# NeuroDiffGym/neurodiffeq

Measured on NVIDIA H100. Metric: collocation-points/sec (residual+grad), higher is better.
Workload: dtype f32

## Files before the change

### neurodiffeq_b200/csrc/pinnjet_common.cuh

```cuda
#pragma once
#include <cuda_runtime.h>
#include <stdint.h>
#include <stdlib.h>
#include "pinnjet_plan.h"

namespace pj {

inline bool pdl_enabled() {
    static const int on = [] {
        const char* e = getenv("PINNJET_PDL");
        return (e && e[0] == '1') ? 1 : 0;
    }();
    return on != 0;
}

template <typename... KArgs, typename... Args>
inline cudaError_t launch_kernel(void (*kern)(KArgs...), dim3 grid, dim3 block, size_t smem, cudaStream_t s, bool dependent,
                                 Args&&... args) {
    cudaLaunchConfig_t cfg = {};
    cfg.gridDim = grid;
    cfg.blockDim = block;
    cfg.dynamicSmemBytes = smem;
    cfg.stream = s;
    cudaLaunchAttribute attr[1];
// ... 149 lines not shown
__device__ __forceinline__ f2 pack2(float x, float y) {
    f2 r;
    asm("mov.b64 %0, {%1, %2};" : "=l"(r) : "f"(x), "f"(y));
    return r;
}
__device__ __forceinline__ float2 unpack2(f2 v) {
    float2 r;
    asm("mov.b64 {%0, %1}, %2;" : "=f"(r.x), "=f"(r.y) : "l"(v));
    return r;
}
__device__ __forceinline__ void ffma2(f2& d, const f2 a, const f2 b) {
    const float2 x = unpack2(a), y = unpack2(b), z = unpack2(d);
    d = pack2(fmaf(x.x, y.x, z.x), fmaf(x.y, y.y, z.y));
}
struct __align__(16) d2 {
    double x, y;
};
__device__ __forceinline__ d2 pack2(double x, double y) { return d2{x, y}; }
__device__ __forceinline__ double2 unpack2(d2 v) { return make_double2(v.x, v.y); }
__device__ __forceinline__ void ffma2(d2& d, const d2 a, const d2 b) { d = d2{fma(a.x, b.x, d.x), fma(a.y, b.y, d.y)}; }

template <typename R> struct Pair;
template <> struct Pair<float> {
    typedef f2 type;
    typedef ulonglong2 row16;
    __device__ static __forceinline__ void fma16(f2& d, const ulonglong2& a, const ulonglong2& b) {
        ffma2(d, a.x, b.x);
        ffma2(d, a.y, b.y);
    }
};
template <> struct Pair<double> {
    typedef d2 type;
    typedef d2 row16;
    __device__ static __forceinline__ void fma16(d2& d, const d2& a, const d2& b) { ffma2(d, a, b); }
};

__device__ __forceinline__ void store2(float* p, float a, float b) { *reinterpret_cast<float2*>(p) = make_float2(a, b); }
__device__ __forceinline__ void store2(double* p, double a, double b) { *reinterpret_cast<double2*>(p) = make_double2(a, b); }
__device__ __forceinline__ void store4(float* p, float a, float b, float c, float d) {
    *reinterpret_cast<float4*>(p) = make_float4(a, b, c, d);
}
__device__ __forceinline__ void store4(double* p, double a, double b, double c, double d) {
    *reinterpret_cast<double2*>(p) = make_double2(a, b);
    *reinterpret_cast<double2*>(p + 2) = make_double2(c, d);
}

template <typename R>
__device__ __forceinline__ R warp_sum(R v) {
#pragma unroll
    for (int o = 16; o > 0; o >>= 1) v += __shfl_xor_sync(0xffffffffu, v, o);
    return v;
}

template <typename R>
__device__ __forceinline__ R pg_reduce_scatter8(const R (&v)[8], int pg_lane) {
    const bool b2 = pg_lane & 4, b1 = pg_lane & 2, b0 = pg_lane & 1;
    R w[4], x[2];
#pragma unroll
    for (int i = 0; i < 4; ++i)
        w[i] = (b2 ? v[i + 4] : v[i]) + __shfl_xor_sync(0xffffffffu, b2 ? v[i] : v[i + 4], 4);
#pragma unroll
    for (int i = 0; i < 2; ++i)
        x[i] = (b1 ? w[i + 2] : w[i]) + __shfl_xor_sync(0xffffffffu, b1 ? w[i] : w[i + 2], 2);
    return (b0 ? x[1] : x[0]) + __shfl_xor_sync(0xffffffffu, b0 ? x[0] : x[1], 1);
}
template <typename R>
__device__ __forceinline__ R pg_reduce_scatter4(const R (&v)[4], int pg_lane) {
    const bool b2 = pg_lane & 4, b1 = pg_lane & 2;
    R w[2];
#pragma unroll
    for (int i = 0; i < 2; ++i)
        w[i] = (b2 ? v[i + 2] : v[i]) + __shfl_xor_sync(0xffffffffu, b2 ? v[i] : v[i + 2], 4);
    R x = (b1 ? w[1] : w[0]) + __shfl_xor_sync(0xffffffffu, b1 ? w[0] : w[1], 2);
    return x + __shfl_xor_sync(0xffffffffu, x, 1);
}

__device__ __forceinline__ float tanh_fast(float x) {
    const float ax = fabsf(x), t = x * x;
    float p = fmaf(-0.006276387721300125f, t, 0.021116213873028755f);
    p = fmaf(p, t, -0.053875137120485306f);
    p = fmaf(p, t, 0.13332924246788025f);
    p = fmaf(p, t, -0.3333333134651184f);
    const float small = fmaf(x * t, p, x);
    float e;
    asm("ex2.approx.ftz.f32 %0, %1;" : "=f"(e) : "f"(fminf(ax, 15.0f) * 2.885390081777927f));
    float r;
    asm("rcp.approx.ftz.f32 %0, %1;" : "=f"(r) : "f"(e + 1.0f));
    const float big = copysignf(fmaf(-2.0f, r, 1.0f), x);
    return ax < 0.6f ? small : big;
}

__device__ __forceinline__ void act_d2(int act, float z0, float& a0, float& s1, float& s2) {
    if (act == PJ_ACT_TANH) {
        a0 = tanh_fast(z0);
        s1 = fmaf(-a0, a0, 1.0f);
        s2 = -2.0f * a0 * s1;
    } else {
        sincosf(z0, &a0, &s1);
        s2 = -a0;
    }
}
__device__ __forceinline__ void act_d2(int act, double z0, double& a0, double& s1, double& s2) {
    if (act == PJ_ACT_TANH) {
        a0 = tanh(z0);
        s1 = fma(-a0, a0, 1.0);
        s2 = -2.0 * a0 * s1;
    } else {
        sincos(z0, &a0, &s1);
        s2 = -a0;
    }
}
__device__ __forceinline__ void sincos_r(float x, float* s, float* c) { sincosf(x, s, c); }
__device__ __forceinline__ void sincos_r(double x, double* s, double* c) { sincos(x, s, c); }

__device__ __forceinline__ float sigmoid_fast(float x) {
    float e;
    asm("ex2.approx.ftz.f32 %0, %1;" : "=f"(e) : "f"(x * -1.4426950408889634f));
    float r;
    asm("rcp.approx.ftz.f32 %0, %1;" : "=f"(r) : "f"(e + 1.0f));
    return r;
}
__device__ __forceinline__ double sigmoid_r(double x) { return 1.0 / (1.0 + exp(-x)); }
__device__ __forceinline__ float sigmoid_r(float x) { return sigmoid_fast(x); }
__device__ __forceinline__ float tanh_r(float x) { return tanh_fast(x); }
__device__ __forceinline__ double tanh_r(double x) { return tanh(x); }
__device__ __forceinline__ float expm1_r(float x) { return expm1f(x); }
__device__ __forceinline__ double expm1_r(double x) { return expm1(x); }
// ... 199 lines not shown

template <int P, int Q, int C>
__device__ __forceinline__ void gemm_rows(float (&acc)[Q][C][P], const float* __restrict__ a_ptr, int RS, int T,
                                          const float* __restrict__ b_ptr, int ldb, int nrows) {
    static_assert(Q % 4 == 0 && (P == 2 || P == 4), "float4 weight rows, float2 / float4 point rows");
    auto load = [&](int k, float (&a)[C][P], float (&b)[Q]) {
        const float* ar = a_ptr + k * RS;
#pragma unroll
        for (int c = 0; c < C; ++c) {
            if constexpr (P == 4) {
                const float4 v = *reinterpret_cast<const float4*>(ar + c * T);
                a[c][0] = v.x;
                a[c][1] = v.y;
                a[c][2] = v.z;
                a[c][3] = v.w;
            } else {
                const float2 v = *reinterpret_cast<const float2*>(ar + c * T);
                a[c][0] = v.x;
                a[c][1] = v.y;
            }
        }
        const float* br = b_ptr + k * ldb;
#pragma unroll
        for (int q4 = 0; q4 < Q / 4; ++q4) {
            const float4 v = *reinterpret_cast<const float4*>(br + 4 * q4);
            b[4 * q4 + 0] = v.x;
            b[4 * q4 + 1] = v.y;
            b[4 * q4 + 2] = v.z;
            b[4 * q4 + 3] = v.w;
        }
    };
    if (nrows <= 0) return;
    float a[C][P], b[Q];
    load(0, a, b);
#pragma unroll 2
    for (int k = 0; k < nrows; ++k) {
        float an[C][P], bn[Q];
        load(min(k + 1, nrows - 1), an, bn);
#pragma unroll
        for (int q = 0; q < Q; ++q)
#pragma unroll
            for (int c = 0; c < C; ++c)
#pragma unroll
                for (int p = 0; p < P; ++p) acc[q][c][p] = fmaf(a[c][p], b[q], acc[q][c][p]);
#pragma unroll
        for (int c = 0; c < C; ++c)
#pragma unroll
            for (int p = 0; p < P; ++p) a[c][p] = an[c][p];
#pragma unroll
        for (int q = 0; q < Q; ++q) b[q] = bn[q];
    }
}

template <typename R, int P, bool SCALAR>
struct GemmAcc {
    typedef typename Pair<R>::type elem;
    static constexpr int n = P / 2;
};
template <int P>
struct GemmAcc<float, P, true> {
    typedef float elem;
    static constexpr int n = P;
};

template <int P, typename PairT>
__device__ __forceinline__ auto pick(const PairT (&v)[P / 2], int p) {
    const auto t = unpack2(v[p >> 1]);
    return (p & 1) ? t.y : t.x;
}
template <int P>
__device__ __forceinline__ float pick(const float (&v)[P], int p) { return v[p]; }

#ifdef PJ_TIMING
#define PJ_T_DECL unsigned long long pj_t_last = clock64(), pj_t_acc[12] = {0, 0, 0, 0, 0, 0, 0, 0, 0, 0, 0, 0};
#define PJ_T_MARK(slot)                              \
    {                                                \
        const unsigned long long now_ = clock64();   \
        pj_t_acc[slot] += now_ - pj_t_last;          \
        pj_t_last = now_;                            \
    }
#define PJ_T_FLUSH(base)                                                           \
    if (blockIdx.x == 0 && threadIdx.x == 0) {                                     \
        for (int i_ = 0; i_ < 12; ++i_) A.dbg[(base) + i_] = (float)pj_t_acc[i_];     \
    }
#else
#define PJ_T_DECL
#define PJ_T_MARK(slot)
#define PJ_T_FLUSH(base)
#endif

struct JobMap {
    int p0, u0, pg_lane;
    __device__ __forceinline__ JobMap(int tid, int T, int P, int Q) {
        const int warp = tid >> 5, lane = tid & 31;
        const int n_pgb = (T / P) >> 3;
        pg_lane = lane & 7;
        p0 = P * ((warp % n_pgb) * 8 + pg_lane);
        u0 = Q * ((warp / n_pgb) * 4 + (lane >> 3));
    }
};

}
```

### neurodiffeq_b200/csrc/pinnjet_k1.cuh

```cuda
#pragma once
#include "pinnjet_common.cuh"
#include "pinnjet_program.cuh"

namespace pj {

template <bool kForward, typename R>
__device__ __forceinline__ void weight_producer(const PjSpec& sp, const KNet* nets, const Plan& pl, const R* __restrict__ pack,
                                                R* ring, uint64_t* full, uint64_t* empty, int my_tiles) {
    const bool resident = kForward ? pl.resident_fwd : pl.resident_bwd;
    const int n_stage = kForward ? pl.n_stage : pl.n_stage_bwd;
    const int tiles = resident ? (my_tiles > 0 ? 1 : 0) : my_tiles;
    int it = 0;
    for (int t = 0; t < tiles; ++t) {
        for (int n = 0; n < sp.n_nets; ++n) {
            const int L = nets[n].n_linear - 1;
            for (int li = 1; li < L; ++li) {
                const int l = kForward ? li : (L - li);
                const int rows = kForward ? pl.hp[n][l] : pl.hp[n][l + 1];
                const int cols = kForward ? pl.hp[n][l + 1] : pl.hp[n][l];
                const R* src = pack + (kForward ? pl.b_wt[n][l] : pl.b_wo[n][l]);
                const int rpc = chunk_elems(sizeof(R)) / cols;
                for (int r0 = 0; r0 < rows; r0 += rpc, ++it) {
                    const int nr = min(rpc, rows - r0);
                    const int stage = it % n_stage;
// ... 103 lines not shown
        }
        for (int b = 0; b < 2; ++b) {
            mbar_init(&yfull[b], 1);
            mbar_init(&yempty[b], 1);
        }
        fence_barrier_init();
    }
    pdl_launch_dependents();
    pdl_wait();
    for (int i = tid; i < pl.small_floats; i += NT_TOTAL) small[i] = __ldg(A.pack + i);
    for (int i = tid; i < A.prog_len; i += NT_TOTAL) prog_s[i] = __ldg(A.prog + i);
    if constexpr (WL > 0)
        for (int i = tid; i < A.prog_w_len; i += NT_TOTAL) progw_s[i] = __ldg(A.prog_w + i);
    __syncthreads();

    if (warp == N_CWARPS) {
        if (lane == 0) weight_producer<true>(sp, A.net, pl, A.pack, ring, full, empty, my_tiles);
        if constexpr (N_SVC == 2) return;
        __syncwarp();
    }
    const int tiles_per_batch = EB / T;
    if (warp == N_CWARPS + N_SVC - 1) {
        const bool train_pw = A.mode == 1;
        R my_sumsq = 0.0f;
        const int n_batches = (my_tiles + tiles_per_batch - 1) / tiles_per_batch;
        for (int b = 0; b < n_batches; ++b) {
            const int buf = b & 1;
            mbar_wait(&yfull[buf], (uint32_t)((b >> 1) & 1));
            const R* yb = ycache + (size_t)buf * sp.n_yrows * EB;
            const int first_iter = b * tiles_per_batch;
            const int npts = min(tiles_per_batch, my_tiles - first_iter) * T;
            for (int bp = lane; bp < npts; bp += 32) {
                const int tl = bp / T, pt = bp - tl * T;
                const long long btile = (long long)blockIdx.x + (long long)(first_iter + tl) * gridDim.x;
                const long long gidx = btile * T + pt;
                R* seed_tile = (train_pw && gidx < ws_points)
                                       ? A.seeds + (gidx / T2) * ((long long)sp.n_yrows * T2) + (gidx % T2) : nullptr;
                if (gidx < A.N) {
                    ProgIOT<R> io{A.coords, gidx, A.N, yb + bp, EB, A.rbar, A.loss_scale, A.u_out, A.r_out, seed_tile, T2};
                    my_sumsq += run_program<32>(prog_s, A.prog_len, slots + lane, io);
                } else if (seed_tile) {
                    for (int r = 0; r < sp.n_yrows; ++r) seed_tile[r * T2] = 0.0f;
                }
            }
            __syncwarp();
            if (lane == 0) mbar_arrive(&yempty[buf]);
        }
        my_sumsq = warp_sum(my_sumsq);
        if (lane == 0) A.loss_part[blockIdx.x] = my_sumsq;
        fold_loss_partials(A.loss_part, gridDim.x, A.sumsq_out, A.ticket, lane);
        return;
    }

    const JobMap jm(tid, T, P, Q);
    const int p0 = jm.p0, u0 = jm.u0;
    RingCursor<R> cur{0, NTC == 128 ? MAX_STAGES : pl.n_stage, NTC == 128 || pl.resident_fwd != 0, full, empty, ring};
    const bool train = A.mode == 1;
    int bslot = 0, batch_idx = 0;
    PJ_T_DECL
    PJ_T_MARK(0)

    for (int iter = 0; iter < my_tiles; ++iter) {
        const long long tile = (long long)blockIdx.x + (long long)iter * gridDim.x;
        const long long base = tile * T;
        if (cur.resident) cur.it = 0;
        if (bslot == 0 && batch_idx >= 2) mbar_wait(&yempty[batch_idx & 1], (uint32_t)(((batch_idx >> 1) - 1) & 1));
        R* yb = ycache + (size_t)(batch_idx & 1) * sp.n_yrows * EB + bslot * T;
        if (iter + 1 < my_tiles) {
            const long long nb = (tile + gridDim.x) * T + p0;
            if (nb < A.N)
                for (int i = 0; i < sp.n_coords; ++i) asm volatile("prefetch.global.L1 [%0];" ::"l"(A.coords[i] + nb));
        }
        const bool rec = train && (base + p0 < ws_points);
        R* zj_tile = rec ? A.zj + ((base + p0) / T2) * pl.zj_tile_floats + (p0 % T2) : nullptr;
        if constexpr (WL > 0) {
            const int NW = sp.n_nets * WL;
            if (tid < T) {
                ProgIOT<R> io{A.coords, min(base + tid, A.N - 1), A.N, nullptr, 0, nullptr, 0.0f, nullptr, nullptr, nullptr, T2};
                io.w_out = wbuf + tid;
                io.w_stride = T;
                run_program<NTC>(progw_s, A.prog_w_len, wslots + tid, io);
            }
            bar_compute<NTC>();
            if (train)
                for (int e = tid; e < NW * T; e += NT_COMPUTE) {
                    const int row = e / T, pt = e - row * T;
                    const long long gp = base + pt;
                    if (gp < ws_points) A.wts[(gp / T2) * ((long long)NW * T2) + row * T2 + (gp % T2)] = wbuf[e];
                }
        }

        for (int n = 0; n < sp.n_nets; ++n) {
            const KNet& net = A.net[n];
            const int L = net.n_linear - 1;
            const int act_kind = net.act;
            const R* wrow = wbuf + n * WL * T + p0;

            {
                const int hp1 = pl.hp[n][1];
                if (u0 < hp1) {
                    const R* wt0 = small + pl.s_wt0[n];
                    const R* b0 = small + pl.s_b[n][0];
                    const R* dzt = small + pl.s_dz[n];
                    R x[PJ_MAX_COORDS][P];
#pragma unroll
                    for (int i = 0; i < PJ_MAX_COORDS; ++i)
                        if (i < net.n_in) {
#pragma unroll
                            for (int p = 0; p < P; ++p) {
                                const long long g = min(base + p0 + p, A.N - 1);
                                x[i][p] = __ldg(A.coords[net.in_coord[i]] + g);
                            }
                        }
                    R* zrow = rec ? zj_tile + pl.zj_off[n][1] : nullptr;
#pragma unroll
                    for (int q = 0; q < Q; ++q) {
                        const int u = u0 + q;
                        R w[PJ_MAX_COORDS];
#pragma unroll
                        for (int i = 0; i < PJ_MAX_COORDS; ++i) w[i] = (i < net.n_in) ? wt0[i * hp1 + u] : 0.0f;
                        R dz[N1 > 0 ? N1 : 1];
#pragma unroll
                        for (int f = 0; f < N1; ++f) dz[f] = dzt[f * hp1 + u];
                        R zq[P][C];
#pragma unroll
                        for (int p = 0; p < P; ++p) {
                            R s = b0[u];
#pragma unroll
                            for (int i = 0; i < PJ_MAX_COORDS; ++i)
                                if (i < net.n_in) s = fma(w[i], x[i][p], s);
                            zq[p][0] = s;
#pragma unroll
                            for (int f = 0; f < N1; ++f) zq[p][1 + f] = dz[f];
#pragma unroll
                            for (int s2 = 0; s2 < N2 + N3; ++s2) zq[p][1 + N1 + s2] = 0.0f;
                        }
                        finish_unit<P, N1, N2, WL, N3, XA>(zq, act_kind, act + u * RS + p0, T, rec ? zrow + u * RS2 : nullptr, T2, wrow);
                    }
                }
            }
            bar_compute<NTC>();
            PJ_T_MARK(1)

            for (int l = 1; l < L; ++l) {
                const int K = pl.hp[n][l], NO = pl.hp[n][l + 1];
                const bool valid = u0 < NO;
                typedef GemmAcc<R, P, SCALAR_ACC> GA;
                typename GA::elem acc[Q][C][GA::n];
#pragma unroll
                for (int q = 0; q < Q; ++q)
#pragma unroll
                    for (int c = 0; c < C; ++c)
#pragma unroll
                        for (int h = 0; h < GA::n; ++h) acc[q][c][h] = typename GA::elem{};
                const int rpc = chunk_elems(sizeof(R)) / NO;
                for (int r0 = 0; r0 < K; r0 += rpc) {
                    const R* chunk = cur.acquire();
                    if (valid) gemm_rows<P, Q, C>(acc, act + r0 * RS + p0, RS, T, chunk + u0, NO, min(rpc, K - r0));
                    cur.release(lane);
                }
                PJ_T_MARK(2)
                bar_compute<NTC>();
                PJ_T_MARK(3)
                if (valid) {
                    const R* bl = small + pl.s_b[n][l];
                    R* zrow = rec ? zj_tile + pl.zj_off[n][l + 1] : nullptr;
#pragma unroll
                    for (int q = 0; q < Q; ++q) {
                        const int u = u0 + q;
                        const R bias = bl[u];
                        R zq[P][C];
#pragma unroll
                        for (int c = 0; c < C; ++c)
#pragma unroll
                            for (int p = 0; p < P; ++p) zq[p][c] = pick<P>(acc[q][c], p) + (c == 0 ? bias : 0.0f);
                        finish_unit<P, N1, N2, WL, N3, XA>(zq, act_kind, act + u * RS + p0, T, rec ? zrow + u * RS2 : nullptr, T2, wrow);
                    }
                }
                bar_compute<NTC>();
                PJ_T_MARK(4)
            }

            {
                const int hpL = pl.hp[n][L], n_out = net.width[net.n_linear];
                const R* wl = small + pl.s_wlt[n];
                const R* bo = small + pl.s_bout[n];
                const int rows = n_out * C;
                for (int e = tid; e < rows * T; e += NT_COMPUTE) {
                    const int pt = e % T, row = e / T, o = row / C, c = row - o * C;
                    const R* ap = act + c * T + pt;
                    const R* wp = wl + o;
                    R s0 = (c == 0) ? bo[o] : 0.0f, s1 = 0.0f, s2 = 0.0f, s3 = 0.0f;
#pragma unroll 2
                    for (int k = 0; k < hpL; k += 4) {
                        s0 = fma(wp[(k + 0) * n_out], ap[(k + 0) * RS], s0);
                        s1 = fma(wp[(k + 1) * n_out], ap[(k + 1) * RS], s1);
                        s2 = fma(wp[(k + 2) * n_out], ap[(k + 2) * RS], s2);
                        s3 = fma(wp[(k + 3) * n_out], ap[(k + 3) * RS], s3);
                    }
                    yb[(net.yrow0 + row) * EB + pt] = (s0 + s1) + (s2 + s3);
                }
            }
            bar_compute<NTC>();
            PJ_T_MARK(5)
        }

        if (++bslot == tiles_per_batch || iter == my_tiles - 1) {
            if (tid == 0) mbar_arrive(&yfull[batch_idx & 1]);
            ++batch_idx;
            bslot = 0;
        }
// ... 23 lines not shown
```

### neurodiffeq_b200/csrc/pinnjet_k2.cuh

```cuda
#pragma once
#include "pinnjet_common.cuh"
#include "pinnjet_k1.cuh"

namespace pj {

constexpr int WJ = 8, WK = 4;

template <typename R>
__device__ __forceinline__ void wgrad_tile(typename Pair<R>::type (&acc)[WJ][WK][1], const R* __restrict__ g_base, int j_step,
                                           const R* __restrict__ z_base, int k_step, int RS, int n_r) {
    typedef typename Pair<R>::row16 row16;
    constexpr int STEP = 16 / sizeof(R);
#pragma unroll 2
    for (int r = 0; r < n_r; r += STEP) {
        row16 gv[WJ], zv[WK];
#pragma unroll
        for (int i = 0; i < WJ; ++i) gv[i] = *reinterpret_cast<const row16*>(g_base + (size_t)i * j_step * RS + r);
#pragma unroll
        for (int i = 0; i < WK; ++i) zv[i] = *reinterpret_cast<const row16*>(z_base + (size_t)i * k_step * RS + r);
#pragma unroll
        for (int i = 0; i < WJ; ++i)
#pragma unroll
            for (int j = 0; j < WK; ++j) Pair<R>::fma16(acc[i][j][0], gv[i], zv[j]);
    }
}
__device__ __forceinline__ void wgrad_tile(float (&acc)[WJ][WK][2], const float* __restrict__ g_base, int j_step,
                                           const float* __restrict__ z_base, int k_step, int RS, int n_r) {
#pragma unroll 2
    for (int r = 0; r < n_r; r += 4) {
        float4 gv[WJ], zv[WK];
#pragma unroll
        for (int i = 0; i < WJ; ++i) gv[i] = *reinterpret_cast<const float4*>(g_base + (size_t)i * j_step * RS + r);
#pragma unroll
        for (int i = 0; i < WK; ++i) zv[i] = *reinterpret_cast<const float4*>(z_base + (size_t)i * k_step * RS + r);
#pragma unroll
        for (int i = 0; i < WJ; ++i)
#pragma unroll
            for (int j = 0; j < WK; ++j) {
                acc[i][j][0] = fmaf(gv[i].x, zv[j].x, acc[i][j][0]);
                acc[i][j][1] = fmaf(gv[i].y, zv[j].y, acc[i][j][1]);
                acc[i][j][0] = fmaf(gv[i].z, zv[j].z, acc[i][j][0]);
                acc[i][j][1] = fmaf(gv[i].w, zv[j].w, acc[i][j][1]);
            }
    }
}
template <typename PairT>
__device__ __forceinline__ auto wgrad_sum(const PairT (&v)[1]) {
    const auto t = unpack2(v[0]);
    return t.x + t.y;
}
__device__ __forceinline__ float wgrad_sum(const float (&v)[2]) { return v[0] + v[1]; }

template <typename R, int NTC, int P, int Q, int N1, int N2, int WL, int N3, bool WIDE, bool XA>
__device__ __forceinline__ void k2_backward_body(const K2ArgsT<R>& A) {
    constexpr int C = 1 + N1 + N2 + N3;
    constexpr bool SCALAR_ACC = sizeof(R) == 4 && N3 == 0;
    constexpr int NT_COMPUTE = NTC, NT_TOTAL = NTC + 32, N_CWARPS = NTC / 32;
    extern __shared__ __align__(128) unsigned char smem[];
    const PjSpec& sp = A.spec;
    const Plan& pl = A.plan;
    R* G = reinterpret_cast<R*>(smem + pl.k2_g0);
    R* G2 = reinterpret_cast<R*>(smem + pl.k2_g1);
    R* Zb = reinterpret_cast<R*>(smem + pl.k2_zb);
    R* ring = reinterpret_cast<R*>(smem + pl.k2_ring);
    R* small = reinterpret_cast<R*>(smem + pl.k2_small);
    R* ybar = reinterpret_cast<R*>(smem + pl.k2_ybar);
    R* sgrad = reinterpret_cast<R*>(smem + pl.k2_sgrad);
    uint64_t* full = reinterpret_cast<uint64_t*>(smem + pl.k2_misc);
    uint64_t* empty = full + MAX_STAGES;
    uint64_t* zfull = empty + MAX_STAGES;

    const int tid = threadIdx.x, warp = tid >> 5, lane = tid & 31;
    const int T = pl.T, RS = pl.RS;
    const int my_tiles = (pl.n_tiles > (int)blockIdx.x) ? (pl.n_tiles - 1 - (int)blockIdx.x) / (int)gridDim.x + 1 : 0;
    R* gpart = A.gpart + (size_t)blockIdx.x * sp.n_theta;

    if (tid == 0) {
        for (int s = 0; s < MAX_STAGES; ++s) {
            mbar_init(&full[s], 1);
            mbar_init(&empty[s], N_CWARPS);
        }
        mbar_init(zfull, 1);
        fence_barrier_init();
    }
    pdl_launch_dependents();
    pdl_wait();
    for (int i = tid; i < pl.small_floats; i += NT_TOTAL) small[i] = __ldg(A.pack + i);
    for (int i = tid; i < pl.sgrad_floats * pl.sgrad_copies; i += NT_TOTAL) sgrad[i] = 0.0f;
    for (long long i = tid; i < sp.n_theta; i += NT_TOTAL) gpart[i] = 0.0f;
    __syncthreads();

    if (warp == N_CWARPS) {
        if (lane == 0) weight_producer<false>(sp, A.net, pl, A.pack, ring, full, empty, my_tiles);
        return;
    }

    const JobMap jm(tid, T, P, Q);
    const int p0 = jm.p0, u0 = jm.u0;
    R* sg = sgrad + (size_t)(warp % ((T / P) >> 3)) * pl.sgrad_floats;
    RingCursor<R> cur{0, pl.n_stage_bwd, pl.resident_bwd != 0, full, empty, ring};
    uint32_t zphase = 0;
    const int kl = lane & 7, jl = lane >> 3;
    PJ_T_DECL
    PJ_T_MARK(0)

    for (int iter = 0; iter < my_tiles; ++iter) {
        const long long tile = (long long)blockIdx.x + (long long)iter * gridDim.x;
        const long long base = tile * T;
        if (cur.resident) cur.it = 0;
        const R* zj_tile = A.zj + tile * pl.zj_tile_floats;
        const R* seed_tile = A.seeds + tile * ((long long)sp.n_yrows * T);

        for (int n = 0; n < sp.n_nets; ++n) {
            const KNet& net = A.net[n];
            const int L = net.n_linear - 1;
            const int act_kind = net.act;
            const int n_out = net.width[net.n_linear];
            const int hpL = pl.hp[n][L];
            R wq[P][WL > 0 ? WL : 1];
#pragma unroll
            for (int p = 0; p < P; ++p)
#pragma unroll
                for (int dd = 0; dd < (WL > 0 ? WL : 1); ++dd)
                    wq[p][dd] = WL > 0 ? __ldg(A.wts + tile * ((long long)sp.n_nets * WL * T) + (n * WL + dd) * T + p0 + p) : 0.0f;

            if (tid == 0) {
                fence_proxy_async();
                const uint32_t bytes = (uint32_t)(hpL * RS) * (uint32_t)sizeof(R);
                mbar_arrive_expect_tx(zfull, bytes);
                tma_bulk_g2s(Zb, zj_tile + pl.zj_off[n][L], bytes, zfull);
            }
            for (int e = tid; e < n_out * C * T; e += NT_COMPUTE) ybar[e] = __ldg(seed_tile + net.yrow0 * T + e);
            bar_compute<NTC>();
            mbar_wait(zfull, zphase);
            zphase ^= 1u;
            PJ_T_MARK(1)

            {
                const R* wlo = small + pl.s_wlo[n];
                if constexpr (!WIDE) if (u0 < hpL) {
                    static_assert(Q == 4, "the gradient reductions below assume 4 units per thread");
                    static_assert(K2_OUT_GROUP == PJ_MAX_NETS, "the first group's reduction below is written for 4 outputs");
                    R gbq[Q], gwq[K2_OUT_GROUP][Q];
#pragma unroll
                    for (int q = 0; q < Q; ++q) {
                        const int u = u0 + q;
                        R gw[K2_OUT_GROUP];
#pragma unroll
                        for (int o = 0; o < K2_OUT_GROUP; ++o) gw[o] = 0.0f;
                        R gb = 0.0f;
#pragma unroll
                        for (int p = 0; p < P; ++p) {
                            const int pt = p0 + p;
                            R z[C], ab[C], a[C], zb[C];
#pragma unroll
                            for (int c = 0; c < C; ++c) {
                                z[c] = Zb[u * RS + c * T + pt];
                                ab[c] = 0.0f;
                            }
#pragma unroll
                            for (int o = 0; o < K2_OUT_GROUP; ++o)
                                if (o < n_out) {
                                    const R w = wlo[o * hpL + u];
#pragma unroll
                                    for (int c = 0; c < C; ++c) ab[c] = fma(w, ybar[(o * C + c) * T + pt], ab[c]);
                                }
                            act_backward<N1, N2, WL, N3, XA>(act_kind, z, ab, a, zb, wq[p]);
#pragma unroll
                            for (int o = 0; o < K2_OUT_GROUP; ++o)
                                if (o < n_out) {
#pragma unroll
                                    for (int c = 0; c < C; ++c) gw[o] = fma(ybar[(o * C + c) * T + pt], a[c], gw[o]);
                                }
                            gb += zb[0];
#pragma unroll
                            for (int c = 0; c < C; ++c) G[u * RS + c * T + pt] = zb[c];
                        }
                        gbq[q] = gb;
#pragma unroll
                        for (int o = 0; o < K2_OUT_GROUP; ++o) gwq[o][q] = gw[o];
                    }
                    const int pl8 = jm.pg_lane, i4 = pl8 & 3;
                    {
                        const R v0[8] = {gbq[0], gbq[1], gbq[2], gbq[3], gwq[0][0], gwq[0][1], gwq[0][2], gwq[0][3]};
                        const R t0 = pg_reduce_scatter8(v0, pl8);
                        if (pl8 < 4) sg[pl.g_b[n][L - 1] + u0 + i4] += t0; else sg[pl.g_wl[n] + u0 + i4] += t0;
                        if (n_out > 1) {
                            const R v1[8] = {gwq[1][0], gwq[1][1], gwq[1][2], gwq[1][3],
                                                 gwq[2][0], gwq[2][1], gwq[2][2], gwq[2][3]};
                            const R t1 = pg_reduce_scatter8(v1, pl8);
                            if (pl8 < 4) sg[pl.g_wl[n] + hpL + u0 + i4] += t1;
                            else if (n_out > 2) sg[pl.g_wl[n] + 2 * hpL + u0 + i4] += t1;
                        }
                        if (n_out > 3) {
                            const R v2[4] = {gwq[3][0], gwq[3][1], gwq[3][2], gwq[3][3]};
                            const R t2 = pg_reduce_scatter4(v2, pl8);
                            if (!(pl8 & 1)) sg[pl.g_wl[n] + 3 * hpL + u0 + (pl8 >> 1)] += t2;
                        }
                    }
                }
                if constexpr (WIDE) if (u0 < hpL) {
                    R gbq[Q];
#pragma unroll
                    for (int q = 0; q < Q; ++q) {
                        const int u = u0 + q;
                        R gb = 0.0f;
#pragma unroll
                        for (int p = 0; p < P; ++p) {
                            const int pt = p0 + p;
                            R z[C], ab[C], a[C], zb[C];
#pragma unroll
                            for (int c = 0; c < C; ++c) {
                                z[c] = Zb[u * RS + c * T + pt];
                                ab[c] = 0.0f;
                            }
                            for (int o = 0; o < n_out; ++o) {
                                const R w = wlo[o * hpL + u];
#pragma unroll
                                for (int c = 0; c < C; ++c) ab[c] = fma(w, ybar[(o * C + c) * T + pt], ab[c]);
                            }
                            act_backward<N1, N2, WL, N3, XA>(act_kind, z, ab, a, zb, wq[p]);
                            gb += zb[0];
#pragma unroll
                            for (int c = 0; c < C; ++c) {
                                G[u * RS + c * T + pt] = zb[c];
                                Zb[u * RS + c * T + pt] = a[c];
                            }
                        }
                        gbq[q] = gb;
                    }
                    const int pl8 = jm.pg_lane, i4 = pl8 & 3;
                    const R tb = pg_reduce_scatter4(gbq, pl8);
                    if (!(pl8 & 1)) sg[pl.g_b[n][L - 1] + u0 + (pl8 >> 1)] += tb;
                    for (int o0 = 0; o0 < n_out; o0 += K2_OUT_GROUP) {
                        R gwq[K2_OUT_GROUP][Q];
#pragma unroll
                        for (int q = 0; q < Q; ++q) {
                            const int u = u0 + q;
                            R gw[K2_OUT_GROUP];
#pragma unroll
                            for (int o = 0; o < K2_OUT_GROUP; ++o) gw[o] = 0.0f;
#pragma unroll
                            for (int p = 0; p < P; ++p) {
                                const int pt = p0 + p;
                                R a[C];
#pragma unroll
                                for (int c = 0; c < C; ++c) a[c] = Zb[u * RS + c * T + pt];
#pragma unroll
                                for (int o = 0; o < K2_OUT_GROUP; ++o)
                                    if (o0 + o < n_out) {
#pragma unroll
                                        for (int c = 0; c < C; ++c) gw[o] = fma(ybar[((o0 + o) * C + c) * T + pt], a[c], gw[o]);
                                    }
                            }
#pragma unroll
                            for (int o = 0; o < K2_OUT_GROUP; ++o) gwq[o][q] = gw[o];
                        }
                        const int row = o0 + (pl8 >> 2);
                        const R v1[8] = {gwq[0][0], gwq[0][1], gwq[0][2], gwq[0][3],
                                             gwq[1][0], gwq[1][1], gwq[1][2], gwq[1][3]};
                        const R t1 = pg_reduce_scatter8(v1, pl8);
                        if (row < n_out) sg[pl.g_wl[n] + row * hpL + u0 + i4] += t1;
                        if (o0 + 2 < n_out) {
                            const R v2[8] = {gwq[2][0], gwq[2][1], gwq[2][2], gwq[2][3],
                                                 gwq[3][0], gwq[3][1], gwq[3][2], gwq[3][3]};
                            const R t2 = pg_reduce_scatter8(v2, pl8);
                            if (row + 2 < n_out) sg[pl.g_wl[n] + (row + 2) * hpL + u0 + i4] += t2;
                        }
                    }
                }
                if (tid < n_out) {
                    R s = 0.0f;
                    for (int pt = 0; pt < T; ++pt) s += ybar[(tid * C) * T + pt];
                    sgrad[pl.g_bout[n] + tid] += s;
                }
            }
            bar_compute<NTC>();
            PJ_T_MARK(2)

            for (int h = L; h >= 2; --h) {
                const int l = h - 1;
                const int HJ = pl.hp[n][h], HK = pl.hp[n][h - 1];
                if (tid == 0) {
                    fence_proxy_async();
                    const uint32_t bytes = (uint32_t)(HK * RS) * (uint32_t)sizeof(R);
                    mbar_arrive_expect_tx(zfull, bytes);
                    tma_bulk_g2s(Zb, zj_tile + pl.zj_off[n][h - 1], bytes, zfull);
                }
                const bool valid = u0 < HK;
                typedef GemmAcc<R, P, SCALAR_ACC> AA;
                typename AA::elem acc[Q][C][AA::n];
#pragma unroll
                for (int q = 0; q < Q; ++q)
#pragma unroll
                    for (int c = 0; c < C; ++c)
#pragma unroll
                        for (int hh = 0; hh < AA::n; ++hh) acc[q][c][hh] = typename AA::elem{};
                const int rpc = chunk_elems(sizeof(R)) / HK;
                for (int r0 = 0; r0 < HJ; r0 += rpc) {
                    const R* chunk = cur.acquire();
                    if (valid) gemm_rows<P, Q, C>(acc, G + r0 * RS + p0, RS, T, chunk + u0, HK, min(rpc, HJ - r0));
                    cur.release(lane);
                }
                PJ_T_MARK(3)
                mbar_wait(zfull, zphase);
                zphase ^= 1u;
                PJ_T_MARK(4)
                if (valid) {
                    R gbq[Q];
#pragma unroll
                    for (int q = 0; q < Q; ++q) {
                        const int u = u0 + q;
                        R gb = 0.0f;
                        R av[P][C], zv[P][C];
#pragma unroll
                        for (int p = 0; p < P; ++p) {
                            R z[C], ab[C];
#pragma unroll
                            for (int c = 0; c < C; ++c) {
                                z[c] = Zb[u * RS + c * T + p0 + p];
                                ab[c] = pick<P>(acc[q][c], p);
                            }
                            act_backward<N1, N2, WL, N3, XA>(act_kind, z, ab, av[p], zv[p], wq[p]);
                            gb += zv[p][0];
                        }
#pragma unroll
                        for (int c = 0; c < C; ++c) {
                            if constexpr (P == 4) {
                                store4(Zb + u * RS + c * T + p0, av[0][c], av[1][c], av[2][c], av[3][c]);
                                store4(G2 + u * RS + c * T + p0, zv[0][c], zv[1][c], zv[2][c], zv[3][c]);
                            } else {
                                store2(Zb + u * RS + c * T + p0, av[0][c], av[1][c]);
                                store2(G2 + u * RS + c * T + p0, zv[0][c], zv[1][c]);
                            }
                        }
                        gbq[q] = gb;
                    }
                    const R tb = pg_reduce_scatter4(gbq, jm.pg_lane);
                    if (!(jm.pg_lane & 1)) sg[pl.g_b[n][h - 2] + u0 + (jm.pg_lane >> 1)] += tb;
                }
                bar_compute<NTC>();
                PJ_T_MARK(5)
                {
                    const int width_j = net.width[h], width_k = net.width[h - 1];
                    const int n_kb = HK / 32, n_jb = HJ / 32;
                    R* gw = gpart + net.w_off[l];
                    for (int wt = warp; wt < n_kb * n_jb; wt += N_CWARPS) {
                        const int jb = (wt / n_kb) * 32, kb = (wt % n_kb) * 32;
                        typedef GemmAcc<R, 2, SCALAR_ACC> WA;
                        typename WA::elem wacc[WJ][WK][WA::n];
#pragma unroll
                        for (int i = 0; i < WJ; ++i)
#pragma unroll
                            for (int jj = 0; jj < WK; ++jj)
#pragma unroll
                                for (int hh = 0; hh < WA::n; ++hh) wacc[i][jj][hh] = typename WA::elem{};
                        wgrad_tile(wacc, G + (size_t)(jb + jl) * RS, 4, Zb + (size_t)(kb + kl) * RS, 8, RS, C * T);
#pragma unroll
                        for (int i = 0; i < WJ; ++i) {
                            const int j = jb + jl + 4 * i;
#pragma unroll
                            for (int jj = 0; jj < WK; ++jj) {
                                const int k = kb + kl + 8 * jj;
                                if (j < width_j && k < width_k) {
                                    atomicAdd(&gw[(size_t)j * width_k + k], wgrad_sum(wacc[i][jj]));
                                }
                            }
                        }
                    }
                }
                bar_compute<NTC>();
                PJ_T_MARK(6)
                R* t = G;
                G = G2;
                G2 = t;
            }

            {
                const int hp1 = pl.hp[n][1];
                if (u0 < hp1) {
                    R x[PJ_MAX_COORDS][P];
#pragma unroll
                    for (int i = 0; i < PJ_MAX_COORDS; ++i)
                        if (i < net.n_in) {
#pragma unroll
                            for (int p = 0; p < P; ++p) {
                                const long long g = min(base + p0 + p, A.N - 1);
                                x[i][p] = __ldg(A.coords[net.in_coord[i]] + g);
                            }
                        }
#pragma unroll
                    for (int q = 0; q < Q; ++q) {
                        const int u = u0 + q;
                        R s0[P];
                        R sf[N1 > 0 ? N1 : 1];
#pragma unroll
                        for (int f = 0; f < N1; ++f) sf[f] = 0.0f;
#pragma unroll
                        for (int p = 0; p < P; ++p) {
                            s0[p] = G[u * RS + p0 + p];
#pragma unroll
                            for (int f = 0; f < N1; ++f) sf[f] += G[u * RS + (1 + f) * T + p0 + p];
                        }
                        R sv[PJ_MAX_COORDS];
#pragma unroll
                        for (int i = 0; i < PJ_MAX_COORDS; ++i) {
                            R s = 0.0f;
                            if (i < net.n_in) {
#pragma unroll
                                for (int p = 0; p < P; ++p) s = fma(s0[p], x[i][p], s);
#pragma unroll
                                for (int f = 0; f < N1; ++f) s = fma(sf[f], R(sp.dir[f][net.in_coord[i]]), s);
                            }
                            sv[i] = s;
                        }
                        if (net.n_in <= 4) {
                            const R v4[4] = {sv[0], sv[1], sv[2], sv[3]};
                            const R t = pg_reduce_scatter4(v4, jm.pg_lane);
                            const int i = jm.pg_lane >> 1;
                            if (!(jm.pg_lane & 1) && i < net.n_in) sg[pl.g_w0[n] + u * net.n_in + i] += t;
                        } else {
                            const R t = pg_reduce_scatter8(sv, jm.pg_lane);
                            if (jm.pg_lane < net.n_in) sg[pl.g_w0[n] + u * net.n_in + jm.pg_lane] += t;
                        }
                    }
                }
            }
            bar_compute<NTC>();
            PJ_T_MARK(7)
        }
    }
    PJ_T_FLUSH(16)

    bar_compute<NTC>();
    for (int n = 0; n < sp.n_nets; ++n) {
        const KNet& net = A.net[n];
        const int L = net.n_linear - 1;
        const int h1 = net.width[1], hL = net.width[L], hpL = pl.hp[n][L], n_out = net.width[net.n_linear];
        auto sgsum = [&](int idx) {
            R v = 0.0f;
            for (int c = 0; c < pl.sgrad_copies; ++c) v += sgrad[(size_t)c * pl.sgrad_floats + idx];
            return v;
        };
        for (int e = tid; e < h1 * net.n_in; e += NT_COMPUTE) gpart[net.w_off[0] + e] += sgsum(pl.g_w0[n] + e);
        for (int hl = 0; hl < L; ++hl)
            for (int e = tid; e < net.width[hl + 1]; e += NT_COMPUTE) gpart[net.b_off[hl] + e] += sgsum(pl.g_b[n][hl] + e);
        for (int e = tid; e < n_out * hL; e += NT_COMPUTE) {
            const int o = e / hL, k = e - o * hL;
            gpart[net.w_off[L] + e] += sgsum(pl.g_wl[n] + o * hpL + k);
        }
        for (int e = tid; e < n_out; e += NT_COMPUTE) gpart[net.b_off[L] + e] += sgsum(pl.g_bout[n] + e);
    }
}

template <int NTC, int MINB, int P, int Q, int N1, int N2, int WL, int N3, bool WIDE>
__global__ void __launch_bounds__(ffma_k2_threads(NTC), MINB) k2_backward_kernel(const __grid_constant__ K2Args A) {
    k2_backward_body<float, NTC, P, Q, N1, N2, WL, N3, WIDE, false>(A);
}
template <int NTC, int MINB, int P, int Q, int N1, int N2, int WL, int N3, bool WIDE>
__global__ void __launch_bounds__(ffma_k2_threads(NTC), MINB) k2_backward_kernel_f64(const __grid_constant__ K2ArgsF64 A) {
    k2_backward_body<double, NTC, P, Q, N1, N2, WL, N3, WIDE, false>(A);
}
template <int NTC, int MINB, int P, int Q, int N1, int N2, int WL, int N3, bool WIDE>
__global__ void __launch_bounds__(ffma_k2_threads(NTC), MINB) k2_backward_kernel_xact(const __grid_constant__ K2Args A) {
    k2_backward_body<float, NTC, P, Q, N1, N2, WL, N3, WIDE, true>(A);
}
template <int NTC, int MINB, int P, int Q, int N1, int N2, int WL, int N3, bool WIDE>
__global__ void __launch_bounds__(ffma_k2_threads(NTC), MINB) k2_backward_kernel_f64_xact(const __grid_constant__ K2ArgsF64 A) {
    k2_backward_body<double, NTC, P, Q, N1, N2, WL, N3, WIDE, true>(A);
}

}
```

Before: 71.75 million.

## Use 3xTF32 tensor-core MMA for hidden-layer and weight-gradient GEMMs in f32

Adds an mma.sync m16n8k8 TF32 path that splits each f32 operand into big and small TF32 parts (3xTF32) to keep close to fp32 accuracy. It is used for the forward and backward hidden-layer GEMMs and for the weight-gradient tiles when the config has 128 compute threads, no third-order channels and at most 6 channels. The warp lane-to-job mapping changes to fit the MMA fragment layout, so the point-group shuffle reductions now take a lane stride. The goal is to move FMA-bound SIMT GEMM work onto tensor cores. In exchange each product costs three MMAs plus split instructions, and register pressure rises.

```diff
diff --git a/neurodiffeq_b200/csrc/pinnjet_common.cuh b/neurodiffeq_b200/csrc/pinnjet_common.cuh
--- a/neurodiffeq_b200/csrc/pinnjet_common.cuh
+++ b/neurodiffeq_b200/csrc/pinnjet_common.cuh
@@ -225,27 +225,27 @@
     return v;
 }
 
-template <typename R>
+template <int S = 1, typename R>
 __device__ __forceinline__ R pg_reduce_scatter8(const R (&v)[8], int pg_lane) {
     const bool b2 = pg_lane & 4, b1 = pg_lane & 2, b0 = pg_lane & 1;
     R w[4], x[2];
 #pragma unroll
     for (int i = 0; i < 4; ++i)
-        w[i] = (b2 ? v[i + 4] : v[i]) + __shfl_xor_sync(0xffffffffu, b2 ? v[i] : v[i + 4], 4);
+        w[i] = (b2 ? v[i + 4] : v[i]) + __shfl_xor_sync(0xffffffffu, b2 ? v[i] : v[i + 4], 4 * S);
 #pragma unroll
     for (int i = 0; i < 2; ++i)
-        x[i] = (b1 ? w[i + 2] : w[i]) + __shfl_xor_sync(0xffffffffu, b1 ? w[i] : w[i + 2], 2);
-    return (b0 ? x[1] : x[0]) + __shfl_xor_sync(0xffffffffu, b0 ? x[0] : x[1], 1);
-}
-template <typename R>
+        x[i] = (b1 ? w[i + 2] : w[i]) + __shfl_xor_sync(0xffffffffu, b1 ? w[i] : w[i + 2], 2 * S);
+    return (b0 ? x[1] : x[0]) + __shfl_xor_sync(0xffffffffu, b0 ? x[0] : x[1], S);
+}
+template <int S = 1, typename R>
 __device__ __forceinline__ R pg_reduce_scatter4(const R (&v)[4], int pg_lane) {
     const bool b2 = pg_lane & 4, b1 = pg_lane & 2;
     R w[2];
 #pragma unroll
     for (int i = 0; i < 2; ++i)
-        w[i] = (b2 ? v[i + 2] : v[i]) + __shfl_xor_sync(0xffffffffu, b2 ? v[i] : v[i + 2], 4);
-    R x = (b1 ? w[1] : w[0]) + __shfl_xor_sync(0xffffffffu, b1 ? w[0] : w[1], 2);
-    return x + __shfl_xor_sync(0xffffffffu, x, 1);
+        w[i] = (b2 ? v[i + 2] : v[i]) + __shfl_xor_sync(0xffffffffu, b2 ? v[i] : v[i + 2], 4 * S);
+    R x = (b1 ? w[1] : w[0]) + __shfl_xor_sync(0xffffffffu, b1 ? w[0] : w[1], 2 * S);
+    return x + __shfl_xor_sync(0xffffffffu, x, S);
 }
 
 __device__ __forceinline__ float tanh_fast(float x) {
@@ -551,6 +551,103 @@
     }
 }
 
+__device__ __forceinline__ void split_tf32(float x, uint32_t& big, uint32_t& small) {
+    big = (__float_as_uint(x) + 0x1000u) & 0xffffe000u;
+    small = __float_as_uint(x - __uint_as_float(big));
+}
+__device__ __forceinline__ void mma_tf32(float (&d)[4], const uint32_t (&a)[4], const uint32_t (&b)[2]) {
+    asm volatile("mma.sync.aligned.m16n8k8.row.col.f32.tf32.tf32.f32 {%0,%1,%2,%3}, {%4,%5,%6,%7}, {%8,%9}, {%0,%1,%2,%3};"
+                 : "+f"(d[0]), "+f"(d[1]), "+f"(d[2]), "+f"(d[3])
+                 : "r"(a[0]), "r"(a[1]), "r"(a[2]), "r"(a[3]), "r"(b[0]), "r"(b[1]));
+}
+__device__ __forceinline__ void mma_tf32x3(float (&d)[4], const uint32_t (&ab)[4], const uint32_t (&as)[4], const uint32_t (&bb)[2],
+                                           const uint32_t (&bs)[2]) {
+    mma_tf32(d, as, bb);
+    mma_tf32(d, ab, bs);
+    mma_tf32(d, ab, bb);
+}
+
+template <typename R, int NTC, int C, int N3>
+constexpr bool mma_gemms() { return sizeof(R) == 4 && N3 == 0 && NTC == 128 && C <= 6; }
+
+template <int P, int C, bool AHEAD = true>
+__device__ __forceinline__ void gemm_rows_mma(float (&acc)[4][C][P], const float* __restrict__ a_ptr, int RS, int T,
+                                              const float* __restrict__ b_ptr, int ldb, int nrows, int lane) {
+    static_assert(P == 2 || P == 4, "float2 / float4 point rows");
+    const int g = lane >> 2, t = lane & 3;
+    const float* ap = a_ptr + 2 * t * RS;
+    const float* bp = b_ptr - 4 * t + 4 * (g >> 1) + (g & 1) + 2 * t * ldb;
+    struct Ops {
+        float a[2][C][P], b[2][2];
+    };
+    auto load = [&](int k0, Ops& o) {
+#pragma unroll
+        for (int i = 0; i < 2; ++i) {
+            const float* ar = ap + (k0 + i) * RS;
+#pragma unroll
+            for (int c = 0; c < C; ++c) {
+                if constexpr (P == 4) {
+                    const float4 v = *reinterpret_cast<const float4*>(ar + c * T);
+                    o.a[i][c][0] = v.x;
+                    o.a[i][c][1] = v.y;
+                    o.a[i][c][2] = v.z;
+                    o.a[i][c][3] = v.w;
+                } else {
+                    const float2 v = *reinterpret_cast<const float2*>(ar + c * T);
+                    o.a[i][c][0] = v.x;
+                    o.a[i][c][1] = v.y;
+                }
+            }
+#pragma unroll
+            for (int ni = 0; ni < 2; ++ni) o.b[ni][i] = bp[(k0 + i) * ldb + 2 * ni];
+        }
+    };
+    if (nrows <= 0) return;
+    float d[C][P / 2][2][4];
+#pragma unroll
+    for (int c = 0; c < C; ++c)
+#pragma unroll
+        for (int h = 0; h < P / 2; ++h)
+#pragma unroll
+            for (int ni = 0; ni < 2; ++ni)
+#pragma unroll
+                for (int e = 0; e < 4; ++e) d[c][h][ni][e] = acc[2 * ni + (e & 1)][c][2 * h + (e >> 1)];
+    Ops cur;
+    if constexpr (AHEAD) load(0, cur);
+#pragma unroll 1
+    for (int k0 = 0; k0 < nrows; k0 += 8) {
+        Ops nxt;
+        if constexpr (AHEAD) load(min(k0 + 8, nrows - 8), nxt);
+        else load(k0, cur);
+        uint32_t bb[2][2], bs[2][2];
+#pragma unroll
+        for (int ni = 0; ni < 2; ++ni)
+#pragma unroll
+            for (int i = 0; i < 2; ++i) split_tf32(cur.b[ni][i], bb[ni][i], bs[ni][i]);
+#pragma unroll
+        for (int c = 0; c < C; ++c)
+#pragma unroll
+            for (int h = 0; h < P / 2; ++h) {
+                uint32_t ab[4], as[4];
+                split_tf32(cur.a[0][c][2 * h], ab[0], as[0]);
+                split_tf32(cur.a[0][c][2 * h + 1], ab[1], as[1]);
+                split_tf32(cur.a[1][c][2 * h], ab[2], as[2]);
+                split_tf32(cur.a[1][c][2 * h + 1], ab[3], as[3]);
+#pragma unroll
+                for (int ni = 0; ni < 2; ++ni) mma_tf32x3(d[c][h][ni], ab, as, bb[ni], bs[ni]);
+            }
+        if constexpr (AHEAD) cur = nxt;
+    }
+#pragma unroll
+    for (int c = 0; c < C; ++c)
+#pragma unroll
+        for (int h = 0; h < P / 2; ++h)
+#pragma unroll
+            for (int ni = 0; ni < 2; ++ni)
+#pragma unroll
+                for (int e = 0; e < 4; ++e) acc[2 * ni + (e & 1)][c][2 * h + (e >> 1)] = d[c][h][ni][e];
+}
+
 template <typename R, int P, bool SCALAR>
 struct GemmAcc {
     typedef typename Pair<R>::type elem;
@@ -588,15 +685,17 @@
 #define PJ_T_FLUSH(base)
 #endif
 
+template <bool MMA = false>
 struct JobMap {
+    static constexpr int PG_STEP = MMA ? 4 : 1;
     int p0, u0, pg_lane;
     __device__ __forceinline__ JobMap(int tid, int T, int P, int Q) {
         const int warp = tid >> 5, lane = tid & 31;
         const int n_pgb = (T / P) >> 3;
-        pg_lane = lane & 7;
+        pg_lane = MMA ? lane >> 2 : lane & 7;
         p0 = P * ((warp % n_pgb) * 8 + pg_lane);
-        u0 = Q * ((warp / n_pgb) * 4 + (lane >> 3));
-    }
-};
-
-}
+        u0 = Q * ((warp / n_pgb) * 4 + (MMA ? lane & 3 : lane >> 3));
+    }
+};
+
+}
diff --git a/neurodiffeq_b200/csrc/pinnjet_k1.cuh b/neurodiffeq_b200/csrc/pinnjet_k1.cuh
--- a/neurodiffeq_b200/csrc/pinnjet_k1.cuh
+++ b/neurodiffeq_b200/csrc/pinnjet_k1.cuh
@@ -179,7 +179,8 @@
         return;
     }
 
-    const JobMap jm(tid, T, P, Q);
+    constexpr bool MMA = mma_gemms<R, NTC, C, N3>();
+    const JobMap<MMA> jm(tid, T, P, Q);
     const int p0 = jm.p0, u0 = jm.u0;
     RingCursor<R> cur{0, NTC == 128 ? MAX_STAGES : pl.n_stage, NTC == 128 || pl.resident_fwd != 0, full, empty, ring};
     const bool train = A.mode == 1;
@@ -283,7 +284,10 @@
                 const int rpc = chunk_elems(sizeof(R)) / NO;
                 for (int r0 = 0; r0 < K; r0 += rpc) {
                     const R* chunk = cur.acquire();
-                    if (valid) gemm_rows<P, Q, C>(acc, act + r0 * RS + p0, RS, T, chunk + u0, NO, min(rpc, K - r0));
+                    if (valid) {
+                        if constexpr (MMA) gemm_rows_mma<P, C, P == 2 && C <= 4>(acc, act + r0 * RS + p0, RS, T, chunk + u0, NO, min(rpc, K - r0), lane);
+                        else gemm_rows<P, Q, C>(acc, act + r0 * RS + p0, RS, T, chunk + u0, NO, min(rpc, K - r0));
+                    }
                     cur.release(lane);
                 }
                 PJ_T_MARK(2)
diff --git a/neurodiffeq_b200/csrc/pinnjet_k2.cuh b/neurodiffeq_b200/csrc/pinnjet_k2.cuh
--- a/neurodiffeq_b200/csrc/pinnjet_k2.cuh
+++ b/neurodiffeq_b200/csrc/pinnjet_k2.cuh
@@ -51,10 +51,56 @@
 }
 __device__ __forceinline__ float wgrad_sum(const float (&v)[2]) { return v[0] + v[1]; }
 
+struct WgradMma {
+    uint32_t a[2][2][4], b[4][2][2];
+    __device__ __forceinline__ void load(const float* __restrict__ g, const float* __restrict__ z, int RS, int r0) {
+        const float* gr = g + r0;
+        const float* zr = z + r0;
+#pragma unroll
+        for (int mi = 0; mi < 2; ++mi) {
+            const float* p = gr + 16 * mi * RS;
+            split_tf32(p[0], a[mi][0][0], a[mi][1][0]);
+            split_tf32(p[8 * RS], a[mi][0][1], a[mi][1][1]);
+            split_tf32(p[4], a[mi][0][2], a[mi][1][2]);
+            split_tf32(p[8 * RS + 4], a[mi][0][3], a[mi][1][3]);
+        }
+#pragma unroll
+        for (int ni = 0; ni < 4; ++ni) {
+            const float* p = zr + 8 * ni * RS;
+            split_tf32(p[0], b[ni][0][0], b[ni][1][0]);
+            split_tf32(p[4], b[ni][0][1], b[ni][1][1]);
+        }
+    }
+};
+__device__ __forceinline__ void wgrad_tile_mma(float (&acc)[2][4][4], const float* __restrict__ g_warp,
+                                               const float* __restrict__ z_warp, int RS, int n_r, int lane) {
+    const int g = lane >> 2, t = lane & 3;
+    const float* gb = g_warp + g * RS + t;
+    const float* zb = z_warp + g * RS + t;
+    WgradMma cur;
+    cur.load(gb, zb, RS, 0);
+#pragma unroll 1
+    for (int r0 = 0; r0 < n_r; r0 += 8) {
+        WgradMma nxt;
+        nxt.load(gb, zb, RS, min(r0 + 8, n_r - 8));
+#pragma unroll
+        for (int mi = 0; mi < 2; ++mi)
+#pragma unroll
+            for (int ni = 0; ni < 4; ++ni) {
+                mma_tf32(acc[mi][ni], cur.a[mi][1], cur.b[ni][0]);
+                mma_tf32(acc[mi][ni], cur.a[mi][0], cur.b[ni][1]);
+                mma_tf32(acc[mi][ni], cur.a[mi][0], cur.b[ni][0]);
+            }
+        cur = nxt;
+    }
+}
+
 template <typename R, int NTC, int P, int Q, int N1, int N2, int WL, int N3, bool WIDE, bool XA>
 __device__ __forceinline__ void k2_backward_body(const K2ArgsT<R>& A) {
     constexpr int C = 1 + N1 + N2 + N3;
     constexpr bool SCALAR_ACC = sizeof(R) == 4 && N3 == 0;
+    constexpr bool MMA = mma_gemms<R, NTC, C, N3>();
+    constexpr int PGS = JobMap<MMA>::PG_STEP;
     constexpr int NT_COMPUTE = NTC, NT_TOTAL = NTC + 32, N_CWARPS = NTC / 32;
     extern __shared__ __align__(128) unsigned char smem[];
     const PjSpec& sp = A.spec;
@@ -95,7 +141,7 @@
         return;
     }
 
-    const JobMap jm(tid, T, P, Q);
+    const JobMap<MMA> jm(tid, T, P, Q);
     const int p0 = jm.p0, u0 = jm.u0;
     R* sg = sgrad + (size_t)(warp % ((T / P) >> 3)) * pl.sgrad_floats;
     RingCursor<R> cur{0, pl.n_stage_bwd, pl.resident_bwd != 0, full, empty, ring};
@@ -183,18 +229,18 @@
                     const int pl8 = jm.pg_lane, i4 = pl8 & 3;
                     {
                         const R v0[8] = {gbq[0], gbq[1], gbq[2], gbq[3], gwq[0][0], gwq[0][1], gwq[0][2], gwq[0][3]};
-                        const R t0 = pg_reduce_scatter8(v0, pl8);
+                        const R t0 = pg_reduce_scatter8<PGS>(v0, pl8);
                         if (pl8 < 4) sg[pl.g_b[n][L - 1] + u0 + i4] += t0; else sg[pl.g_wl[n] + u0 + i4] += t0;
                         if (n_out > 1) {
                             const R v1[8] = {gwq[1][0], gwq[1][1], gwq[1][2], gwq[1][3],
                                                  gwq[2][0], gwq[2][1], gwq[2][2], gwq[2][3]};
-                            const R t1 = pg_reduce_scatter8(v1, pl8);
+                            const R t1 = pg_reduce_scatter8<PGS>(v1, pl8);
                             if (pl8 < 4) sg[pl.g_wl[n] + hpL + u0 + i4] += t1;
                             else if (n_out > 2) sg[pl.g_wl[n] + 2 * hpL + u0 + i4] += t1;
                         }
                         if (n_out > 3) {
                             const R v2[4] = {gwq[3][0], gwq[3][1], gwq[3][2], gwq[3][3]};
-                            const R t2 = pg_reduce_scatter4(v2, pl8);
+                            const R t2 = pg_reduce_scatter4<PGS>(v2, pl8);
                             if (!(pl8 & 1)) sg[pl.g_wl[n] + 3 * hpL + u0 + (pl8 >> 1)] += t2;
                         }
                     }
@@ -230,7 +276,7 @@
                         gbq[q] = gb;
                     }
                     const int pl8 = jm.pg_lane, i4 = pl8 & 3;
-                    const R tb = pg_reduce_scatter4(gbq, pl8);
+                    const R tb = pg_reduce_scatter4<PGS>(gbq, pl8);
                     if (!(pl8 & 1)) sg[pl.g_b[n][L - 1] + u0 + (pl8 >> 1)] += tb;
                     for (int o0 = 0; o0 < n_out; o0 += K2_OUT_GROUP) {
                         R gwq[K2_OUT_GROUP][Q];
@@ -259,12 +305,12 @@
                         const int row = o0 + (pl8 >> 2);
                         const R v1[8] = {gwq[0][0], gwq[0][1], gwq[0][2], gwq[0][3],
                                              gwq[1][0], gwq[1][1], gwq[1][2], gwq[1][3]};
-                        const R t1 = pg_reduce_scatter8(v1, pl8);
+                        const R t1 = pg_reduce_scatter8<PGS>(v1, pl8);
                         if (row < n_out) sg[pl.g_wl[n] + row * hpL + u0 + i4] += t1;
                         if (o0 + 2 < n_out) {
                             const R v2[8] = {gwq[2][0], gwq[2][1], gwq[2][2], gwq[2][3],
                                                  gwq[3][0], gwq[3][1], gwq[3][2], gwq[3][3]};
-                            const R t2 = pg_reduce_scatter8(v2, pl8);
+                            const R t2 = pg_reduce_scatter8<PGS>(v2, pl8);
                             if (row + 2 < n_out) sg[pl.g_wl[n] + (row + 2) * hpL + u0 + i4] += t2;
                         }
                     }
@@ -299,7 +345,10 @@
                 const int rpc = chunk_elems(sizeof(R)) / HK;
                 for (int r0 = 0; r0 < HJ; r0 += rpc) {
                     const R* chunk = cur.acquire();
-                    if (valid) gemm_rows<P, Q, C>(acc, G + r0 * RS + p0, RS, T, chunk + u0, HK, min(rpc, HJ - r0));
+                    if (valid) {
+                        if constexpr (MMA) gemm_rows_mma<P, C>(acc, G + r0 * RS + p0, RS, T, chunk + u0, HK, min(rpc, HJ - r0), lane);
+                        else gemm_rows<P, Q, C>(acc, G + r0 * RS + p0, RS, T, chunk + u0, HK, min(rpc, HJ - r0));
+                    }
                     cur.release(lane);
                 }
                 PJ_T_MARK(3)
@@ -336,7 +385,7 @@
                         }
                         gbq[q] = gb;
                     }
-                    const R tb = pg_reduce_scatter4(gbq, jm.pg_lane);
+                    const R tb = pg_reduce_scatter4<PGS>(gbq, jm.pg_lane);
                     if (!(jm.pg_lane & 1)) sg[pl.g_b[n][h - 2] + u0 + (jm.pg_lane >> 1)] += tb;
                 }
                 bar_compute<NTC>();
@@ -347,23 +396,36 @@
                     R* gw = gpart + net.w_off[l];
                     for (int wt = warp; wt < n_kb * n_jb; wt += N_CWARPS) {
                         const int jb = (wt / n_kb) * 32, kb = (wt % n_kb) * 32;
-                        typedef GemmAcc<R, 2, SCALAR_ACC> WA;
-                        typename WA::elem wacc[WJ][WK][WA::n];
-#pragma unroll
-                        for (int i = 0; i < WJ; ++i)
-#pragma unroll
-                            for (int jj = 0; jj < WK; ++jj)
-#pragma unroll
-                                for (int hh = 0; hh < WA::n; ++hh) wacc[i][jj][hh] = typename WA::elem{};
-                        wgrad_tile(wacc, G + (size_t)(jb + jl) * RS, 4, Zb + (size_t)(kb + kl) * RS, 8, RS, C * T);
-#pragma unroll
-                        for (int i = 0; i < WJ; ++i) {
-                            const int j = jb + jl + 4 * i;
-#pragma unroll
-                            for (int jj = 0; jj < WK; ++jj) {
-                                const int k = kb + kl + 8 * jj;
-                                if (j < width_j && k < width_k) {
-                                    atomicAdd(&gw[(size_t)j * width_k + k], wgrad_sum(wacc[i][jj]));
+                        if constexpr (MMA) {
+                            float wacc[2][4][4] = {};
+                            wgrad_tile_mma(wacc, G + (size_t)jb * RS, Zb + (size_t)kb * RS, RS, C * T, lane);
+#pragma unroll
+                            for (int mi = 0; mi < 2; ++mi)
+#pragma unroll
+                                for (int ni = 0; ni < 4; ++ni)
+#pragma unroll
+                                    for (int e = 0; e < 4; ++e) {
+                                        const int j = jb + 16 * mi + (lane >> 2) + 8 * (e >> 1);
+                                        const int k = kb + 8 * ni + 2 * (lane & 3) + (e & 1);
+                                        if (j < width_j && k < width_k) atomicAdd(&gw[(size_t)j * width_k + k], wacc[mi][ni][e]);
+                                    }
+                        } else {
+                            typedef GemmAcc<R, 2, SCALAR_ACC> WA;
+                            typename WA::elem wacc[WJ][WK][WA::n];
+#pragma unroll
+                            for (int i = 0; i < WJ; ++i)
+#pragma unroll
+                                for (int jj = 0; jj < WK; ++jj)
+#pragma unroll
+                                    for (int hh = 0; hh < WA::n; ++hh) wacc[i][jj][hh] = typename WA::elem{};
+                            wgrad_tile(wacc, G + (size_t)(jb + jl) * RS, 4, Zb + (size_t)(kb + kl) * RS, 8, RS, C * T);
+#pragma unroll
+                            for (int i = 0; i < WJ; ++i) {
+                                const int j = jb + jl + 4 * i;
+#pragma unroll
+                                for (int jj = 0; jj < WK; ++jj) {
+                                    const int k = kb + kl + 8 * jj;
+                                    if (j < width_j && k < width_k) atomicAdd(&gw[(size_t)j * width_k + k], wgrad_sum(wacc[i][jj]));
                                 }
                             }
                         }
@@ -416,11 +478,11 @@
                         }
                         if (net.n_in <= 4) {
                             const R v4[4] = {sv[0], sv[1], sv[2], sv[3]};
-                            const R t = pg_reduce_scatter4(v4, jm.pg_lane);
+                            const R t = pg_reduce_scatter4<PGS>(v4, jm.pg_lane);
                             const int i = jm.pg_lane >> 1;
                             if (!(jm.pg_lane & 1) && i < net.n_in) sg[pl.g_w0[n] + u * net.n_in + i] += t;
                         } else {
-                            const R t = pg_reduce_scatter8(sv, jm.pg_lane);
+                            const R t = pg_reduce_scatter8<PGS>(sv, jm.pg_lane);
                             if (jm.pg_lane < net.n_in) sg[pl.g_w0[n] + u * net.n_in + jm.pg_lane] += t;
                         }
                     }
```

Measured after the change: 81.87 million, median of 6. +14.1%, better.
